# soasme/LTX-Video-GPUPoor

Measured on AMD Instinct MI355X. Metric: denoise-steps/sec + VAE-decode frames/sec, LTX-Video 768x512x97f at 1/8 GPU, higher is better.
Workload: dtype bf16

## Files before the change

### ltx-video-gpupoor_amd/ltxmi/attention.py

```python
from enum import Enum, auto
from typing import Optional

import torch
from torch import nn

from . import ff_mx8, lora, ops
from .attention_seam import pay_attention
from .derived import DerivedOwner, cache_key

BF16 = torch.bfloat16


FUSE_CROSS_ATTENTION_Q = True


class SkipLayerStrategy(Enum):
    AttentionSkip = auto()
    AttentionValues = auto()
    Residual = auto()
    TransformerBlock = auto()


def reshape_hidden_states(hidden_states, latent_frames):
    return hidden_states.reshape(hidden_states.shape[0], latent_frames, -1, hidden_states.shape[-1])


def restore_hidden_states_shape(hidden_states):
    return hidden_states.reshape(hidden_states.shape[0], -1, hidden_states.shape[-1])


class RMSNorm(nn.Module):

    def __init__(self, dim, eps: float, elementwise_affine: bool = True):
        super().__init__()
        self.eps = eps
        self.dim = dim
        if elementwise_affine:
            self.weight = nn.Parameter(torch.ones(dim))
        else:
            self.register_parameter("weight", None)


class _NoAffineLayerNorm(nn.Module):
    def __init__(self, dim, eps: float, elementwise_affine: bool = False):
        super().__init__()
        if elementwise_affine:
            raise NotImplementedError("ltxmi: standardisation norms with affine parameters are not on this path")
        self.eps = eps
        self.dim = dim


class GELUProj(nn.Module):

    def __init__(self, dim_in, dim_out, approximate="tanh", bias=True):
        super().__init__()
        self.proj = nn.Linear(dim_in, dim_out, bias=bias)
        self.approximate = approximate


class FeedForward(nn.Module):

    def __init__(self, dim, dim_out=None, mult=4, dropout=0.0, activation_fn="geglu", final_dropout=False,
                 inner_dim=None, bias=True):
        super().__init__()
        if activation_fn != "gelu-approximate":
            raise NotImplementedError(f"ltxmi: activation_fn '{activation_fn}' is not on this path "
# ... 126 lines not shown
                ops.rmsnorm_rope_(q2, attn.q_norm.weight, attn.q_norm.eps, cos, sin, period)
                ops.rmsnorm_rope_(k2, attn.k_norm.weight, attn.k_norm.eps, cos, sin, period)
            Lk = N
            q4 = qkv.view(B, N, 3, H, dh)[:, :, 0]
            k4 = qkv.view(B, N, 3, H, dh)[:, :, 1]
            v4 = qkv.view(B, N, 3, H, dh)[:, :, 2]
            v3 = qkv.view(B, N, 3 * D)[:, :, 2 * D:]
        else:
            Bk, Lk, _ = encoder_hidden_states.shape
            fuse_q = FUSE_CROSS_ATTENTION_Q and D % 64 == 0 and bool(ops.attention_fuses_qnorm(B, H, N, Lk, dh, attention_mask is not None))
            ss = torch.empty((B * N, D // 64), dtype=torch.float32, device=x2.device) if fuse_q else None
            q2 = ops.gemm(x2, attn.to_q.weight, attn.to_q.bias, rowsumsq=ss, rowsumsq_cols=D if fuse_q else 0,
                          **lora.pair(attn, "q", x2))
            ehs = encoder_hidden_states
            kv = None
            ready = attn.__dict__.get("_text_kv_ready")
            if ready is not None:
                full, full_key, kv_full, ready_epoch = ready
                row_bytes = full.stride(0) * full.element_size()
                off = ehs.data_ptr() - full.data_ptr()
                if (row_bytes > 0 and off >= 0 and off % row_bytes == 0 and ehs.shape[1:] == full.shape[1:]
                        and off // row_bytes + Bk <= full.shape[0] and ehs.dtype == full.dtype and ehs.is_contiguous()
                        and cache_key((full,)) == full_key and ready_epoch == lora.epoch(attn)):
                    r0 = off // row_bytes
                    kv = kv_full[r0 * Lk:(r0 + Bk) * Lk]
            if kv is None:
                def project():
                    e2 = ehs.reshape(Bk * Lk, -1)
                    kv = ops.gemm(e2, wkv, bkv, **lora.pair(attn, "kv", e2))
                    ops.rmsnorm_rope_(kv[:, :D], attn.k_norm.weight, attn.k_norm.eps)
                    return kv
                kv = attn.derived("text_kv", 4, True).get((ehs, wkv, attn.k_norm.weight), (lora.epoch(attn),), project,
                                                    enabled=ops.STEP_INVARIANT_CACHING)
            if fuse_q:
                q_fused = ((ops.rowsumsq_rstd(ss, D, attn.q_norm.eps), attn.q_norm.weight, attn.q_norm.eps), None)
            else:
                ops.rmsnorm_rope_(q2, attn.q_norm.weight, attn.q_norm.eps)
            q4 = q2.view(B, N, H, dh)
            k4 = kv.view(Bk, Lk, 2, H, dh)[:, :, 0]
            v4 = kv.view(Bk, Lk, 2, H, dh)[:, :, 1]
            v3 = kv.view(Bk, Lk, 2 * D)[:, :, D:]

        host_mask = _host_mask(skip_layer_mask) if skip_layer_mask is not None else None
        skip_attention = (host_mask is not None and skip_layer_strategy == SkipLayerStrategy.AttentionValues
                          and len(host_mask) == 1 and host_mask[0] == 0)
        if skip_attention:
            a3 = v3.contiguous()
        else:
            mask4 = None
            if attention_mask is not None:
                if attention_mask.dim() != 3 or attention_mask.shape[1] != 1:
                    raise NotImplementedError("ltxmi.AttnProcessor2_0: attention_mask must be a [B,1,Lk] bias")
                mask4 = attention_mask.reshape(B, 1, 1, Lk)
            a4 = self.attend([q4, k4, v4], is_cross, attention_mask=mask4, softmax_scale=attn.scale,
                             q_norm=q_fused[0] if q_fused else None, rope=q_fused[1] if q_fused else None)
            a3 = a4.view(B, N, D)
            if host_mask is not None and any(m != 1.0 for m in host_mask):
                m_dev = skip_layer_mask.reshape(B).to(torch.float32)
                if skip_layer_strategy == SkipLayerStrategy.AttentionValues:
                    ops.stg_blend_(a3, v3, m_dev)
                elif skip_layer_strategy == SkipLayerStrategy.AttentionSkip:
                    ops.stg_blend_(a3, hidden_states, m_dev)

        w_o, b_o = attn.to_out[0].weight, attn.to_out[0].bias
        if fused_residual is not None:
            residual, gate_table, gate_temb, rpg = fused_residual
            ops.gemm(a3.reshape(B * N, D), w_o, b_o, out=residual.reshape(B * N, -1),
                     epilogue=ops.EPI_GATE_RESIDUAL, residual=residual.reshape(B * N, -1),
                     gate_table=gate_table, gate_temb=gate_temb, rows_per_group=rpg,
                     **lora.pair(attn, "out", a3.reshape(B * N, D)))
            return residual
        out = ops.gemm(a3.reshape(B * N, D), w_o, b_o, **lora.pair(attn, "out", a3.reshape(B * N, D))).view(B, N, -1)
        if attn.residual_connection or attn.rescale_output_factor != 1.0:
            raise NotImplementedError("ltxmi.AttnProcessor2_0: residual_connection / rescale_output_factor")
        return out


class BasicTransformerBlock(nn.Module):

    def __init__(self, dim, num_attention_heads, attention_head_dim, dropout=0.0, cross_attention_dim=None,
                 activation_fn="geglu", num_embeds_ada_norm=None, attention_bias=False, only_cross_attention=False,
                 double_self_attention=False, upcast_attention=False, norm_elementwise_affine=True,
                 adaptive_norm="single_scale_shift", standardization_norm="layer_norm", norm_eps=1e-5,
                 qk_norm=None, final_dropout=False, attention_type="default", ff_inner_dim=None, ff_bias=True,
                 attention_out_bias=True, use_tpu_flash_attention=False, use_rope=False):
        super().__init__()
        if adaptive_norm != "single_scale_shift" or only_cross_attention or double_self_attention:
            raise NotImplementedError("ltxmi.BasicTransformerBlock: only the AdaLN-Zero "
                                      "(single_scale_shift) self+cross block is on this path")
        assert standardization_norm in ("layer_norm", "rms_norm")
        self.adaptive_norm = adaptive_norm
        self.norm_kind = ops.NORM_RMS if standardization_norm == "rms_norm" else ops.NORM_LAYER
        make_norm = RMSNorm if standardization_norm == "rms_norm" else _NoAffineLayerNorm
        if norm_elementwise_affine:
            raise NotImplementedError("ltxmi.BasicTransformerBlock: norm_elementwise_affine=True is not on this path")
        self.norm1 = make_norm(dim, eps=norm_eps, elementwise_affine=False)
        self.attn1 = Attention(query_dim=dim, heads=num_attention_heads, dim_head=attention_head_dim,
                               dropout=dropout, bias=attention_bias, cross_attention_dim=None,
                               out_bias=attention_out_bias, qk_norm=qk_norm, use_rope=use_rope)
        if cross_attention_dim is not None:
            self.attn2 = Attention(query_dim=dim, cross_attention_dim=cross_attention_dim,
                                   heads=num_attention_heads, dim_head=attention_head_dim, dropout=dropout,
                                   bias=attention_bias, out_bias=attention_out_bias, qk_norm=qk_norm,
                                   use_rope=use_rope)
        else:
            self.attn2 = None
        self.norm2 = make_norm(dim, norm_eps, False)
        self.ff = FeedForward(dim, dropout=dropout, activation_fn=activation_fn, final_dropout=final_dropout,
# ... 122 lines not shown
```

### ltx-video-gpupoor_amd/ltxmi/attention_seam.py

```python
import torch

from . import ops
from .derived import DerivedCache


def _key_bias_from_mask(attention_mask, B, Lk):
    m = attention_mask
    if m.dim() != 4 or m.shape[0] != B or m.shape[-1] != Lk:
        raise ValueError(f"pay_attention: attention_mask must be [B, 1|Lq, 1|H, Lk], got {tuple(m.shape)}")
    for d in (1, 2):
        if m.shape[d] != 1 and m.stride(d) != 0:
            raise NotImplementedError(
                "pay_attention: only key biases broadcast over queries and heads are supported "
                f"(mask dim {d} has size {m.shape[d]} with stride {m.stride(d)})")
    return _BIAS_CACHE.get((m,), (), lambda: m[:, 0, 0, :].to(torch.float32).contiguous())


_BIAS_CACHE = DerivedCache(4)


@torch.compiler.disable()
def pay_attention(qkv_list, dropout_p=0., softmax_scale=None, causal=False, window_size=(-1, -1),
                  deterministic=False, version=None, force_attention=None, attention_mask=None,
                  cross_attn=False, q_lens=None, k_lens=None, q_norm=None, rope=None):
    q, k, v = qkv_list
    qkv_list.clear()
    if (q_norm is not None or rope is not None) and (q_lens is not None or k_lens is not None):
        raise NotImplementedError("pay_attention: q_norm / rope on load with q_lens / k_lens")
    if causal or tuple(window_size) != (-1, -1) or dropout_p != 0.:
        raise NotImplementedError("pay_attention: causal / windowed / dropout attention is not on this path")
    if force_attention not in (None, "sdpa"):
        raise NotImplementedError(f"pay_attention: backend '{force_attention}' does not exist here (single HIP backend)")
    out_dtype = q.dtype
    if v.dtype != torch.bfloat16:
        raise TypeError(f"pay_attention: bf16 only on this path, got {v.dtype}")
    q = q.to(v.dtype)
    k = k.to(v.dtype)
    b, lq, lk = q.size(0), q.size(1), k.size(1)
    final_padding = 0

    if b > 1 and k_lens is not None:
        assert attention_mask is None and q_lens is None
        k_lens = [int(x) for x in k_lens]
        chunk_sizes, k_sizes = [], []
        cur, cnt = k_lens[0], 1
        for kl in k_lens[1:]:
            if kl == cur:
                cnt += 1
            else:
                chunk_sizes.append(cnt)
                k_sizes.append(cur)
                cur, cnt = kl, 1
        chunk_sizes.append(cnt)
        k_sizes.append(cur)
        if len(chunk_sizes) > 1 or k_lens[0] != k.shape[1]:
            outs = []
            for sq, sk, sv, sz in zip(torch.split(q, chunk_sizes), torch.split(k, chunk_sizes),
                                      torch.split(v, chunk_sizes), k_sizes):
                outs.append(pay_attention([sq, sk[:, :sz], sv[:, :sz]], softmax_scale=softmax_scale))
            return torch.cat(outs, dim=0)
    elif q_lens is not None or k_lens is not None:
        assert b == 1
        szq = int(q_lens[0]) if q_lens is not None else lq
        szk = int(k_lens[0]) if k_lens is not None else lk
        final_padding = lq - szq
        q, k, v = q[:, :szq], k[:, :szk], v[:, :szk]

    bias = None if attention_mask is None else _key_bias_from_mask(attention_mask, b, k.size(1))
    x = ops.attention(q, k, v, key_bias=bias, softmax_scale=softmax_scale, q_norm=q_norm, rope=rope)
    x = x.type(out_dtype)
    if final_padding > 0:
        x = torch.cat([x, torch.empty((x.shape[0], final_padding, *x.shape[-2:]), dtype=x.dtype, device=x.device)], 1)
    return x
```

### ltx-video-gpupoor_amd/ltxmi/ops.py

```python
import ctypes
import math

import torch

from . import _lib, _lib_mx, derived
from ._lib import lib, check

BF16 = torch.bfloat16


def _header(*names):
    return tuple(_lib.CONSTANTS["LTXMI_" + n] for n in names)


EPI_NONE, EPI_GELU_TANH, EPI_SILU, EPI_GATE_RESIDUAL = _header("EPI_NONE", "EPI_GELU_TANH", "EPI_SILU", "EPI_GATE_RESIDUAL")
NORM_RMS, NORM_LAYER = _header("NORM_RMS", "NORM_LAYER")


def _stream():
    return ctypes.c_void_p(torch.cuda.current_stream().cuda_stream)


_watch = None
_events = {}


def watch_launches(keys):
    global _watch
    _watch = set(keys) if keys else None
    _events.clear()


_redo_counter = None


def count_attention_redos(counter):
    global _redo_counter
    _redo_counter = counter


def launch_times_ms():
    return {k: [a.elapsed_time(b) for a, b in v] for k, v in _events.items()}


def _prof_begin(key, key2=None):
    if _watch is None:
        return None
    if key not in _watch:
        if key2 is None or key2 not in _watch:
            return None
        key = key2
    e0, e1 = torch.cuda.Event(enable_timing=True), torch.cuda.Event(enable_timing=True)
    e0.record()
    return key, e0, e1


def _prof_end(tok):
    if tok is not None:
# ... 134 lines not shown

def _norm_modulate(what, f32in, x, out, eps, kind, scale_table, scale_temb, shift_table, shift_temb, rows_per_group):
    if f32in:
        _chk_f32(x, what)
    _chk_bf16(None if f32in else x, out, scale_table, scale_temb, shift_table, shift_temb)
    x2, rows, ldx = _rows(x)
    o2, orows, ldy = _rows(out)
    D = x2.shape[1]
    if f32in and (orows != rows or o2.shape[1] != D):
        raise ValueError(f"ltxmi.{what}: out must have x's rows and channels")
    if scale_temb.stride(0) != shift_temb.stride(0):
        raise ValueError(f"ltxmi.{what}: scale/shift tables must share a row stride")
    entry = lib.ltxmi_norm_modulate_f32in_bf16 if f32in else lib.ltxmi_norm_modulate_bf16
    check(entry(_ptr(x2), ldx, _ptr(o2), ldy, rows, D, eps, kind, _ptr(scale_table), _ptr(scale_temb), _ptr(shift_table),
                _ptr(shift_temb), scale_temb.stride(0), rows_per_group, _stream()),
          "ltxmi_norm_modulate_f32in_bf16" if f32in else "ltxmi_norm_modulate_bf16")
    return out


def norm_modulate(x, out, eps, kind, scale_table, scale_temb, shift_table, shift_temb, rows_per_group):
    return _norm_modulate("norm_modulate", False, x, out, eps, kind, scale_table, scale_temb, shift_table, shift_temb,
                          rows_per_group)


def norm_modulate_f32in(x, out, eps, kind, scale_table, scale_temb, shift_table, shift_temb, rows_per_group):
    return _norm_modulate("norm_modulate_f32in", True, x, out, eps, kind, scale_table, scale_temb, shift_table, shift_temb,
                          rows_per_group)


def gate_residual_f32_(h, y, gate_table=None, gate_temb=None, rows_per_group=1, round_product=0, h_bf16=None):
    _chk_f32(h, "gate_residual_f32_")
    _chk_bf16(y, gate_table, gate_temb, h_bf16)
    h2, rows, ldh = _rows(h)
    y2, yrows, ldy = _rows(y)
    D = h2.shape[1]
    if yrows != rows or y2.shape[1] != D:
        raise ValueError("ltxmi.gate_residual_f32_: y must have h's rows and channels")
    if (gate_table is None) != (gate_temb is None):
        raise ValueError("ltxmi.gate_residual_f32_: gate_table and gate_temb go together")
    gate_ld = 0
    if gate_temb is not None:
        gate_ld = gate_temb.stride(0) if gate_temb.dim() == 2 else 0
    b2, ldb = None, 0
    if h_bf16 is not None:
        b2, brows, ldb = _rows(h_bf16)
        if brows != rows or b2.shape[1] != D:
            raise ValueError("ltxmi.gate_residual_f32_: h_bf16 must have h's rows and channels")
    check(lib.ltxmi_gate_residual_f32(_ptr(h2), ldh, _ptr(y2), ldy, rows, D, _ptr(gate_table), _ptr(gate_temb), gate_ld,
                                      rows_per_group, int(round_product), _ptr(b2), ldb, _stream()),
          "ltxmi_gate_residual_f32")
    return h


def rmsnorm_rope_(x, weight, eps, cos=None, sin=None, rope_period=0, rstd_of=None):
    _chk_bf16(x, weight, cos, sin)
    x2, rows, ldx = _rows(x)
    D = x2.shape[1]
    ld_tab = 0
    if cos is not None:
        if cos.dim() != 2 or cos.shape != sin.shape or cos.stride(0) != sin.stride(0):
            raise ValueError("ltxmi.rmsnorm_rope_: cos/sin must be matching 2-D tables")
        ld_tab = cos.stride(0)
        rope_period = rope_period or cos.shape[0]
    if rstd_of is not None:
        ss, norm_dim, norm_eps, out = rstd_of
        if ss.dtype != torch.float32 or out.dtype != torch.float32 or ss.dim() != 2 or ss.shape[0] != rows or \
                ss.stride(1) != 1 or out.shape != (rows,) or not out.is_contiguous():
            raise ValueError("ltxmi.rmsnorm_rope_: rstd_of needs fp32 sums [rows, blocks] and a contiguous fp32 out [rows]")
        check(lib.ltxmi_rmsnorm_rope_rstd_bf16(_ptr(x2), ldx, rows, D, _ptr(weight), eps, _ptr(cos), _ptr(sin), ld_tab,
                                               rope_period, _ptr(ss), ss.stride(0), ss.shape[1], norm_dim, norm_eps,
                                               _ptr(out), _stream()), "ltxmi_rmsnorm_rope_rstd_bf16")
        return x
    check(lib.ltxmi_rmsnorm_rope_bf16(_ptr(x2), ldx, rows, D, _ptr(weight), eps, _ptr(cos), _ptr(sin), ld_tab,
                                      rope_period, _stream()), "ltxmi_rmsnorm_rope_bf16")
    return x


def rowsumsq_rstd(ss, norm_dim, eps, out=None):
    if ss.dtype != torch.float32 or ss.dim() != 2 or ss.stride(1) != 1 or not ss.is_cuda:
        raise ValueError("ltxmi.rowsumsq_rstd: expected CUDA fp32 sums [rows, blocks]")
    rows = ss.shape[0]
    out = torch.empty((rows,), dtype=torch.float32, device=ss.device) if out is None else out
    check(lib.ltxmi_rowsumsq_rstd_f32(_ptr(ss), ss.stride(0), ss.shape[1], rows, norm_dim, eps, _ptr(out), _stream()),
          "ltxmi_rowsumsq_rstd_f32")
    return out


def attention_fuses_qnorm(B, H, Lq, Lk, dh, has_key_bias=False):
    return bool(lib.ltxmi_attention_fuses_qnorm(B, H, Lq, Lk, dh, int(has_key_bias)))


def attention_kernel_id(B, H, Lq, Lk, dh, has_key_bias=False, k_stride_l=None, v_stride_l=None):
    ks = 3 * H * dh if k_stride_l is None else k_stride_l
    vs = ks if v_stride_l is None else v_stride_l
    return int(lib.ltxmi_attention_kernel_id(B, H, Lq, Lk, dh, int(has_key_bias), ks, vs))


def _attn_shared(a, what, cuda_bias, dims, q, k, v, out, key_bias, softmax_scale):
    B, H, Lq, Lk, dh = dims
    a.q, a.q_stride_b, a.q_stride_l = q.data_ptr(), q.stride(0), q.stride(1)
    a.k, a.k_stride_b, a.k_stride_l = k.data_ptr(), k.stride(0), k.stride(1)
    a.v, a.v_stride_b, a.v_stride_l = v.data_ptr(), v.stride(0), v.stride(1)
    a.o, a.o_stride_b, a.o_stride_l = out.data_ptr(), out.stride(0), out.stride(1)
    if key_bias is not None:
        if key_bias.dtype != torch.float32 or key_bias.shape != (B, Lk) or key_bias.stride(1) != 1 \
                or (cuda_bias and not key_bias.is_cuda):
            raise ValueError(f"ltxmi.{what}: key_bias must be {'a CUDA ' if cuda_bias else ''}fp32 [B, Lk]")
        a.key_bias, a.bias_stride_b = key_bias.data_ptr(), key_bias.stride(0)
    a.B, a.H, a.Lq, a.Lk, a.head_dim = B, H, Lq, Lk, dh
    a.softmax_scale = softmax_scale


def _chk_attn_qkv(what, q, k, v, out):
    _chk_bf16(q, k, v, out)
    B, Lq, H, dh = q.shape
    for t in (q, k, v):
        if t.stride(3) != 1 or t.stride(2) != dh:
            raise ValueError(f"ltxmi.{what}: (heads, head_dim) must be contiguous")
    return B, H, Lq, k.shape[1], dh


# ... 7 lines not shown
    if out.dim() != 4 or out.stride(3) != 1 or out.stride(2) != dh:
        raise ValueError("ltxmi.attention: out must be 4-D with (heads, head_dim) contiguous")
    a = _lib.AttnArgs()
    if out_segments is not None:
        seg_len, seg_stride = out_segments
        if seg_len <= 0 or Lq % seg_len != 0 or tuple(out.shape) != (B, seg_len, H, dh):
            raise ValueError(f"ltxmi.attention: out_segments=({seg_len}, {seg_stride}) needs Lq={Lq} to be a multiple of the "
                             f"segment and out to be segment 0's [B, segment, H, dh] view, got {tuple(out.shape)}")
        a.o_segment_len, a.o_stride_segment = seg_len, seg_stride
    elif tuple(out.shape) != (B, Lq, H, dh):
        raise ValueError(f"ltxmi.attention: out must be [B, Lq, H, dh] = {(B, Lq, H, dh)}, got {tuple(out.shape)}")
    _attn_shared(a, "attention", False, dims, q, k, v, out, key_bias,
                 softmax_scale if softmax_scale is not None else 1.0 / math.sqrt(dh))
    if q_norm is not None:
        ss, w, eps = q_norm
        nb = H * dh // 64
        _chk_bf16(w)
        if ss.dim() == 1:
            if ss.dtype != torch.float32 or ss.shape != (B * Lq,) or ss.stride(0) != 1 or not ss.is_cuda:
                raise ValueError("ltxmi.attention: q_norm row factors must be a contiguous fp32 [B*Lq]")
            a.q_rstd, a.q_rstd_stride_b, a.q_rstd_stride_l = ss.data_ptr(), Lq, 1
        else:
            if ss.dtype != torch.float32 or ss.dim() != 2 or ss.shape != (B * Lq, nb) or ss.stride(1) != 1:
                raise ValueError("ltxmi.attention: q_norm row sums must be fp32 [B*Lq, H*dh/64]")
            a.q_rowsumsq, a.q_rowsumsq_stride_b, a.q_rowsumsq_stride_l = ss.data_ptr(), Lq * ss.stride(0), ss.stride(0)
            a.q_rowsumsq_blocks = nb
        a.q_norm_weight, a.q_norm_eps = w.data_ptr(), eps
        if rope is not None:
            cos, sin, period = rope
            _chk_bf16(cos, sin)
            if period not in (Lq, B * Lq) or cos.stride(0) != sin.stride(0) or cos.stride(1) != 1:
                raise ValueError("ltxmi.attention: rope tables must be [Lq or B*Lq, H*dh] with one row stride")
            a.rope_cos, a.rope_sin = cos.data_ptr(), sin.data_ptr()
            a.rope_stride_l = cos.stride(0)
            a.rope_stride_b = 0 if period == Lq else Lq * cos.stride(0)
    elif rope is not None:
        raise ValueError("ltxmi.attention: rope needs q_norm")
    if redo_counter is None:
        redo_counter = _redo_counter
    if redo_counter is not None:
        if redo_counter.dtype != torch.int32 or redo_counter.numel() != 1 or not redo_counter.is_cuda:
            raise ValueError("ltxmi.attention: redo_counter must be a CUDA int32 tensor of one element")
        a.redo_counter = redo_counter.data_ptr()
    a.force_exact = int(bool(force_exact))
    if return_lse or lse is not None:
        if lse is None:
            lse = torch.empty((B, H, Lq), dtype=torch.float32, device=q.device)
        _chk_lse(lse, B, H, Lq, "ltxmi.attention: lse")
        a.lse, a.lse_stride_b, a.lse_stride_h = lse.data_ptr(), lse.stride(0), lse.stride(1)
    tok = _prof_begin(("attention", B, H, Lq, Lk, dh))
    check(lib.ltxmi_attention_fwd_bf16(ctypes.byref(a), _stream()), "ltxmi_attention_fwd_bf16")
    _prof_end(tok)
    return (out, lse) if lse is not None else out


def _chk_lse(lse, B, H, Lq, what):
    if lse.dtype != torch.float32 or not lse.is_cuda or tuple(lse.shape) != (B, H, Lq) or lse.stride(2) != 1:
        raise ValueError(f"{what} must be a CUDA fp32 [B, H, Lq] = {(B, H, Lq)} tensor with contiguous tokens")


def attention_merge(outs, lses, out=None, return_lse=False, lse=None):
    n = len(outs)
    if n != len(lses) or not 2 <= n <= _lib.ATTN_MERGE_MAX:
        raise ValueError(f"ltxmi.attention_merge: {n} outputs / {len(lses)} lse tensors, need 2 .. {_lib.ATTN_MERGE_MAX} of each")
    _chk_bf16(*outs, out)
    B, Lq, H, dh = outs[0].shape
    if out is None:
        out = torch.empty((B, Lq, H, dh), dtype=BF16, device=outs[0].device)
    a = _lib.AttnMergeArgs()
    a.n = n
    for i, (o, l) in enumerate(zip(outs, lses)):
        if tuple(o.shape) != (B, Lq, H, dh) or o.stride(3) != 1 or o.stride(2) != dh:
            raise ValueError("ltxmi.attention_merge: partial outputs must be [B, Lq, H, dh] with (heads, head_dim) contiguous")
        _chk_lse(l, B, H, Lq, f"ltxmi.attention_merge: lses[{i}]")
        a.o_part[i], a.o_part_stride_b[i], a.o_part_stride_l[i] = o.data_ptr(), o.stride(0), o.stride(1)
        a.lse_part[i], a.lse_part_stride_b[i], a.lse_part_stride_h[i] = l.data_ptr(), l.stride(0), l.stride(1)
    if tuple(out.shape) != (B, Lq, H, dh) or out.stride(3) != 1 or out.stride(2) != dh:
        raise ValueError("ltxmi.attention_merge: out must be [B, Lq, H, dh] with (heads, head_dim) contiguous")
    a.o, a.o_stride_b, a.o_stride_l = out.data_ptr(), out.stride(0), out.stride(1)
    if return_lse or lse is not None:
        if lse is None:
            lse = torch.empty((B, H, Lq), dtype=torch.float32, device=out.device)
        _chk_lse(lse, B, H, Lq, "ltxmi.attention_merge: lse")
        a.lse, a.lse_stride_b, a.lse_stride_h = lse.data_ptr(), lse.stride(0), lse.stride(1)
    a.B, a.H, a.Lq, a.head_dim = B, H, Lq, dh
    check(lib.ltxmi_attention_merge_bf16(ctypes.byref(a), _stream()), "ltxmi_attention_merge_bf16")
    return (out, lse) if lse is not None else out


def qkv_norm_rope_pack(qkv, B, Nl, D, P, q_weight, k_weight, eps, cos=None, sin=None, rope_period=0, out=None):
    _chk_bf16(qkv, q_weight, k_weight, cos, sin, out)
    x2, rows, ld = _rows(qkv)
    if rows != B * Nl or x2.shape[1] != 3 * D:
        raise ValueError("ltxmi.qkv_norm_rope_pack: qkv must be [B*Nl, 3D]")
    if out is None:
        out = torch.empty((P, Nl, B, 3, D // P), dtype=BF16, device=qkv.device)
    if not out.is_contiguous() or out.numel() != rows * 3 * D:
        raise ValueError("ltxmi.qkv_norm_rope_pack: out must be a contiguous [P, Nl, B, 3, D/P] buffer")
    ld_tab = cos.stride(0) if cos is not None else 0
    check(lib.ltxmi_qkv_norm_rope_pack_bf16(_ptr(x2), ld, B, Nl, D, P, _ptr(q_weight), _ptr(k_weight), eps, _ptr(cos),
                                            _ptr(sin), ld_tab, rope_period, _ptr(out), _stream()),
          "ltxmi_qkv_norm_rope_pack_bf16")
    return out


def stg_blend_grouped_(a, v, m_f32):
# ... 560 lines not shown
```

Measured before the change: 16.50.

## Add cross-attention kernel that skips masked key tiles, plus shared-rope rmsnorm path

Adds a dedicated cross-attention kernel for head_dim 64 and short text keys. A small kernel counts, per batch, how many 64-key tiles hold unmasked keys, and that count is cached per bias tensor. The attention kernel loads only those tiles into shared memory and folds the q RMS-norm into its loads, so padded text tokens cost no matmul work. A separate RMSNorm+RoPE variant is also added that reuses rope tables when the row count is a multiple of the rope period. Both paths are new native kernels and bring risks: edge cases around the discard threshold, and a bias cache keyed on tensor identity.

```diff
diff --git a/include/ltxmi_dit.h b/include/ltxmi_dit.h
--- /dev/null
+++ b/include/ltxmi_dit.h
@@ -0,0 +1,41 @@
+#ifndef LTXMI_DIT_H
+#define LTXMI_DIT_H
+
+#include "ltxmi.h"
+
+#ifdef __cplusplus
+extern "C" {
+#endif
+
+#define LTXMI_DIT_VERSION "1"
+#define LTXMI_KEY_TILE 64
+#define LTXMI_KEY_DISCARD_AT -9000
+#define LTXMI_CROSS_TILES_MAX_KEYS 256
+
+int ltxmi_key_tile_count_f32(const float* key_bias, int64_t bias_stride_b, int32_t B, int32_t Lk, int32_t* key_tiles,
+                             void* stream);
+
+typedef struct ltxmi_cross_tiles_args {
+    const void* q; int64_t q_stride_b, q_stride_l;
+    const void* k; int64_t k_stride_b, k_stride_l;
+    const void* v; int64_t v_stride_b, v_stride_l;
+    void*       o; int64_t o_stride_b, o_stride_l;
+    const float* key_bias; int64_t bias_stride_b;
+    const int32_t* key_tiles;
+    const float* q_rstd; int64_t q_rstd_stride_b, q_rstd_stride_l;
+    const void* q_norm_weight;
+    int32_t B, H, Lq, Lk, head_dim;
+    float softmax_scale;
+} ltxmi_cross_tiles_args;
+
+int ltxmi_attention_cross_tiles_bf16(const ltxmi_cross_tiles_args* args, void* stream);
+
+int ltxmi_rmsnorm_rope_shared_bf16(void* x, int64_t ldx, int32_t B, int32_t N, int32_t D, const void* weight, float eps,
+                                   const void* cos_tab, const void* sin_tab, int64_t ld_tab, const float* rowsumsq,
+                                   int64_t rowsumsq_ld, int32_t rowsumsq_blocks, int32_t norm_dim, float norm_eps,
+                                   float* rstd_out, void* stream);
+
+#ifdef __cplusplus
+}
+#endif
+#endif
diff --git a/ltx-video-gpupoor_amd/csrc/attention_cross_tiles.hip b/ltx-video-gpupoor_amd/csrc/attention_cross_tiles.hip
--- /dev/null
+++ b/ltx-video-gpupoor_amd/csrc/attention_cross_tiles.hip
@@ -0,0 +1,318 @@
+#include "attention.h"
+#include "../../include/ltxmi_dit.h"
+
+namespace ltxmi {
+
+namespace cross_tiles {
+
+#ifndef LTXMI_XATTN_STAGGER
+#define LTXMI_XATTN_STAGGER 32
+#endif
+
+constexpr int DH = 64;
+constexpr int KV_TILE = LTXMI_KEY_TILE;
+constexpr int MAX_TILES = LTXMI_CROSS_TILES_MAX_KEYS / KV_TILE;
+constexpr int ROW_BYTES = DH * 2;
+constexpr int TILE_BYTES = KV_TILE * DH * 2;
+constexpr int K_OFF = 0, V_OFF = MAX_TILES * TILE_BYTES, BIAS_OFF = 2 * MAX_TILES * TILE_BYTES;
+constexpr int SCR_OFF = BIAS_OFF + MAX_TILES * KV_TILE * 16;
+constexpr int SCR_BYTES = 32 * 64;
+constexpr int QW_OFF = SCR_OFF + 4 * SCR_BYTES;
+constexpr int SMEM = QW_OFF + DH * 2;
+constexpr int ROWS_PER_IT = 128;
+constexpr float LOG2E = 1.4426950408889634f;
+
+__device__ __forceinline__ int k_swz(int row) { return (row >> 1) & 7; }
+
+template <int NT>
+__device__ __forceinline__ void attend(const AttnParams& p, char* smem, int b, int head, int row_begin, int row_end,
+                                       int stagger_from) {
+    const int tid = threadIdx.x;
+    const int lane = tid & 63;
+    const int wave = __builtin_amdgcn_readfirstlane(tid >> 6);
+    const int r = lane & 31, hh = lane >> 5;
+    const int n_it = (row_end - row_begin + ROWS_PER_IT - 1) / ROWS_PER_IT;
+
+    const uint16_t* qb = p.q + (int64_t)b * p.q_sb + head * DH;
+    const uint16_t* kb_ = p.k + (int64_t)b * p.k_sb + head * DH;
+    const uint16_t* vb = p.v + (int64_t)b * p.v_sb + head * DH;
+    uint16_t* ob = p.o + (int64_t)b * p.o_sb + head * DH;
+
+    {
+        u32x4 kreg[NT][2], vreg[NT][2];
+#pragma unroll
+        for (int t = 0; t < NT; ++t) {
+#pragma unroll
+            for (int i = 0; i < 2; ++i) {
+                const int c = tid + 256 * i;
+                int key = t * KV_TILE + (c >> 3);
+                key = key < p.Lk ? key : p.Lk - 1;
+                kreg[t][i] = *(const u32x4*)(kb_ + (int64_t)key * p.k_sl + (c & 7) * 8);
+                vreg[t][i] = *(const u32x4*)(vb + (int64_t)key * p.v_sl + (c & 7) * 8);
+            }
+        }
+        if (tid < NT * KV_TILE) {
+            float bv = ATTN_BIAS_FLOOR;
+            if (tid < p.Lk) bv = fmaxf(p.bias[(int64_t)b * p.bias_sb + tid] * (LOG2E / p.scale_log2e), ATTN_BIAS_FLOOR);
+            const __bf16 hi = (__bf16)bv;
+            const __bf16 lo = (__bf16)(bv - (float)hi);
+            u32x4 w = {0u, 0u, 0u, 0u};
+            w[0] = (uint32_t)__builtin_bit_cast(uint16_t, hi) | ((uint32_t)__builtin_bit_cast(uint16_t, lo) << 16);
+            *(u32x4*)(smem + BIAS_OFF + tid * 16) = w;
+        }
+#pragma unroll
+        for (int t = 0; t < NT; ++t) {
+#pragma unroll
+            for (int i = 0; i < 2; ++i) {
+                const int c = tid + 256 * i;
+                const int key = c >> 3, dc = c & 7;
+                *(u32x4*)(smem + K_OFF + t * TILE_BYTES + key * ROW_BYTES + ((dc ^ k_swz(key)) << 4)) = kreg[t][i];
+                *(u32x4*)(smem + V_OFF + t * TILE_BYTES + ((key >> 3) * 2 + (dc >> 2)) * 512 + (key & 7) * 64 + (dc & 3) * 16) = vreg[t][i];
+            }
+        }
+    }
+    if (tid < 8) *(u32x4*)(smem + QW_OFF + tid * 16) = *(const u32x4*)(p.q_w + head * DH + tid * 8);
+    __syncthreads();
+
+    const int k_rd0 = r * ROW_BYTES, k_rd1 = (32 + r) * ROW_BYTES;
+    const int k_sw0 = k_swz(r);
+    const int v_rd = attn_vt_offset(lane);
+    const bf16x8 ones = attn_ones_operand(lane);
+    const float c = p.scale_log2e;
+    char* scr = smem + SCR_OFF + wave * SCR_BYTES;
+
+    bf16x8 qraw[4], qf[4];
+    float q_rstd = 0.f;
+    auto load_q = [&](int it) {
+        const int row = row_begin + it * ROWS_PER_IT + wave * 32 + r;
+        const int q_ld = row < p.Lq ? row : p.Lq - 1;
+#pragma unroll
+        for (int s = 0; s < 4; ++s) qraw[s] = *(const bf16x8*)(qb + (int64_t)q_ld * p.q_sl + 16 * s + 8 * hh);
+        q_rstd = p.q_rstd[(int64_t)b * p.q_rstd_sb + (int64_t)q_ld * p.q_rstd_sl];
+    };
+    auto finish_q = [&]() {
+#pragma unroll
+        for (int s = 0; s < 4; ++s) {
+            const bf16x8 wv = *(const bf16x8*)(smem + QW_OFF + (16 * s + 8 * hh) * 2);
+#pragma unroll
+            for (int e = 0; e < 8; ++e) qf[s][e] = (__bf16)((float)qraw[s][e] * q_rstd * (float)wv[e]);
+        }
+    };
+    load_q(0);
+    finish_q();
+    if (n_it > 1) load_q(1);
+    if (blockIdx.x >= (unsigned)stagger_from) __builtin_amdgcn_s_sleep(LTXMI_XATTN_STAGGER);
+
+    for (int it = 0; it < n_it; ++it) {
+        const int q0 = row_begin + it * ROWS_PER_IT + wave * 32;
+
+        constexpr int NG = 2 * NT;
+        f32x16 sT[NG];
+        bf16x8 kfr[5];
+        bf16x8 qaug;
+        {
+            uint32_t w0 = hh == 0 ? 0x3f803f80u : 0u, w1 = 0u;
+            asm volatile("" : "+v"(w0), "+v"(w1));
+            const u32x4 w = {w0, w1, w1, w1};
+            qaug = __builtin_bit_cast(bf16x8, w);
+        }
+        auto read_k1 = [&](int g, int j) {
+            if (j == 0) {
+                kfr[0] = *(const bf16x8*)(smem + BIAS_OFF + (32 * g + r) * 16);
+            } else {
+                const char* ks = smem + K_OFF + (g >> 1) * TILE_BYTES + ((g & 1) ? k_rd1 : k_rd0);
+                kfr[j] = *(const bf16x8*)(ks + (((2 * (j - 1) + hh) ^ k_sw0) << 4));
+            }
+        };
+        auto max3 = [](float a, float b2, float c3) { return fmaxf(fmaxf(a, b2), c3); };
+        float mt = -INFINITY;
+        auto group_max = [&](int g) {
+            const f32x16& x = sT[g];
+            const float a = max3(x[0], x[1], x[2]), b2 = max3(x[3], x[4], x[5]), c2 = max3(x[6], x[7], x[8]);
+            const float d2 = max3(x[9], x[10], x[11]), e2 = max3(x[12], x[13], x[14]);
+            mt = max3(max3(a, b2, c2), max3(d2, e2, x[15]), mt);
+            asm volatile("" : "+v"(mt));
+        };
+#pragma unroll
+        for (int j = 0; j < 5; ++j) read_k1(0, j);
+#pragma unroll
+        for (int g = 0; g < NG; ++g) {
+#pragma unroll
+            for (int j = 0; j < 5; ++j) {
+                if (j == 0) {
+                    const f32x16 z16 = {0.f, 0.f, 0.f, 0.f, 0.f, 0.f, 0.f, 0.f, 0.f, 0.f, 0.f, 0.f, 0.f, 0.f, 0.f, 0.f};
+                    sT[g] = __builtin_amdgcn_mfma_f32_32x32x16_bf16(kfr[0], qaug, z16, 0, 0, 0);
+                } else {
+                    sT[g] = __builtin_amdgcn_mfma_f32_32x32x16_bf16(kfr[j], qf[j - 1], sT[g], 0, 0, 0);
+                }
+                if (g + 1 < NG) read_k1(g + 1, j);
+                __builtin_amdgcn_sched_barrier(0);
+            }
+            if (g >= 1) group_max(g - 1);
+        }
+        if (it + 1 < n_it) finish_q();
+        if (it + 2 < n_it) load_q(it + 2);
+        group_max(NG - 1);
+        mt = attn_lane_half_max(mt);
+        const float nmc = -mt * c;
+
+        f32x16 oT[2];
+        f32x4 lT;
+        const f32x16 z16 = {0.f, 0.f, 0.f, 0.f, 0.f, 0.f, 0.f, 0.f, 0.f, 0.f, 0.f, 0.f, 0.f, 0.f, 0.f, 0.f};
+        const f32x4 z4 = {0.f, 0.f, 0.f, 0.f};
+        auto read_v = [&](int t, int sp, bf16x8 (&dst)[2]) {
+            const char* vs = smem + V_OFF + t * TILE_BYTES + v_rd;
+#pragma unroll
+            for (int d = 0; d < 2; ++d)
+                dst[d] = attn_vt_fragment<DH>(vs + (2 * sp * 2 + d) * 512);
+        };
+        auto make_p = [&](int t, int sp2, bf16x8& dst) {
+            const f32x16& x = sT[2 * t + (sp2 >> 1)];
+            const f32x2 c2v = {c, c}, m2v = {nmc, nmc};
+#pragma unroll
+            for (int e = 0; e < 8; e += 2) {
+                const f32x2 y = f32x2{x[8 * (sp2 & 1) + e], x[8 * (sp2 & 1) + e + 1]} * c2v + m2v;
+                dst[e] = (__bf16)fast_exp2(y[0]);
+                dst[e + 1] = (__bf16)fast_exp2(y[1]);
+            }
+            asm volatile("" : "+v"(dst));
+        };
+        bf16x8 pfr[2][4], vfr[2][2];
+#pragma unroll
+        for (int sp = 0; sp < 4; ++sp) make_p(0, sp, pfr[0][sp]);
+        read_v(0, 0, vfr[0]);
+#pragma unroll
+        for (int t = 0; t < NT; ++t) {
+#pragma unroll
+            for (int sp = 0; sp < 4; ++sp) {
+                const int st = 4 * t + sp;
+                if (st + 1 < 4 * NT) read_v((st + 1) >> 2, (st + 1) & 3, vfr[(st + 1) & 1]);
+                const bf16x8& pf = pfr[t & 1][sp];
+                lT = __builtin_amdgcn_mfma_f32_16x16x32_bf16(ones, pf, st == 0 ? z4 : lT, 0, 0, 0);
+                oT[0] = __builtin_amdgcn_mfma_f32_32x32x16_bf16(vfr[st & 1][0], pf, st == 0 ? z16 : oT[0], 0, 0, 0);
+                oT[1] = __builtin_amdgcn_mfma_f32_32x32x16_bf16(vfr[st & 1][1], pf, st == 0 ? z16 : oT[1], 0, 0, 0);
+                if (t + 1 < NT) make_p(t + 1, sp, pfr[(t + 1) & 1][sp]);
+                __builtin_amdgcn_sched_barrier(0);
+            }
+        }
+
+        const float l0 = __shfl(lT[0], r & 15, 64), l1v = __shfl(lT[1], r & 15, 64);
+        const float lrow = (r & 16) ? l1v : l0;
+        const float inv = 1.0f / lrow;
+#pragma unroll
+        for (int d = 0; d < 2; ++d) {
+#pragma unroll
+            for (int g = 0; g < 4; ++g) {
+                u32x2 w;
+                w[0] = pack_bf16(oT[d][4 * g + 0] * inv, oT[d][4 * g + 1] * inv);
+                w[1] = pack_bf16(oT[d][4 * g + 2] * inv, oT[d][4 * g + 3] * inv);
+                *(u32x2*)(scr + r * 64 + ((g ^ (r & 3)) << 4) + hh * 8) = w;
+            }
+#pragma unroll
+            for (int t2 = 0; t2 < 2; ++t2) {
+                const int row = t2 * 16 + (lane >> 2), chunk = lane & 3;
+                const u32x4 w = *(const u32x4*)(scr + row * 64 + ((chunk ^ (row & 3)) << 4));
+                if (q0 + row < row_end) *(u32x4*)(ob + (int64_t)(q0 + row) * p.o_sl + 32 * d + chunk * 8) = w;
+            }
+        }
+    }
+}
+
+__global__ __launch_bounds__(256, 2) void attn_cross_tiles_kernel(AttnParams p, const int* __restrict__ key_tiles, int groups,
+                                                                  int rows_per_group, int stagger_from) {
+    extern __shared__ __attribute__((aligned(16))) char smem[];
+    const int work = xcd_work_id();
+    const int bh = work / groups, grp = work % groups;
+    const int b = bh / p.H, head = bh % p.H;
+    const int row_begin = grp * rows_per_group;
+    const int row_end = min(p.Lq, row_begin + rows_per_group);
+    if (row_begin >= row_end) return;
+    const int full = (p.Lk + KV_TILE - 1) / KV_TILE;
+    const int nt = min(max(__builtin_amdgcn_readfirstlane(key_tiles[b]), 1), full);
+    switch (nt) {
+        case 1: attend<1>(p, smem, b, head, row_begin, row_end, stagger_from); break;
+        case 2: attend<2>(p, smem, b, head, row_begin, row_end, stagger_from); break;
+        case 3: attend<3>(p, smem, b, head, row_begin, row_end, stagger_from); break;
+        default: attend<4>(p, smem, b, head, row_begin, row_end, stagger_from); break;
+    }
+}
+
+__global__ __launch_bounds__(64) void key_tile_count_kernel(const float* __restrict__ bias, int64_t bias_sb, int Lk,
+                                                            int* __restrict__ key_tiles) {
+    const int b = blockIdx.x, lane = threadIdx.x;
+    int last = -1;
+    for (int j = lane; j < Lk; j += 64) {
+        const uint32_t bits = __float_as_uint(bias[(int64_t)b * bias_sb + j]);
+        const bool nan = (bits & 0x7fffffffu) > 0x7f800000u;
+        if (nan || __uint_as_float(bits) > (float)LTXMI_KEY_DISCARD_AT) last = j;
+    }
+#pragma unroll
+    for (int o = 32; o > 0; o >>= 1) last = max(last, __shfl_xor(last, o, 64));
+    if (lane == 0) key_tiles[b] = last >= 0 ? last / KV_TILE + 1 : (Lk + KV_TILE - 1) / KV_TILE;
+}
+
+}
+
+}
+
+using namespace ltxmi;
+
+extern "C" int ltxmi_key_tile_count_f32(const float* key_bias, int64_t bias_stride_b, int32_t B, int32_t Lk, int32_t* key_tiles,
+                                        void* stream) {
+    LTXMI_REQUIRE(key_bias && key_tiles, LTXMI_ERR_INVALID_ARG, "ltxmi_key_tile_count_f32: NULL argument");
+    LTXMI_REQUIRE(B > 0 && Lk > 0, LTXMI_ERR_INVALID_ARG, "ltxmi_key_tile_count_f32: non-positive size B=%d Lk=%d", B, Lk);
+    LTXMI_REQUIRE(B == 1 || bias_stride_b >= Lk, LTXMI_ERR_INVALID_ARG,
+                  "ltxmi_key_tile_count_f32: bias_stride_b=%lld is shorter than a row of Lk=%d", (long long)bias_stride_b, Lk);
+    LTXMI_REQUIRE(((((uintptr_t)key_bias) | ((uintptr_t)key_tiles)) & 3) == 0, LTXMI_ERR_INVALID_ARG,
+                  "ltxmi_key_tile_count_f32: key_bias and key_tiles must be 4-byte aligned");
+    hipLaunchKernelGGL(cross_tiles::key_tile_count_kernel, dim3((unsigned)B), dim3(64), 0, (hipStream_t)stream, key_bias,
+                       bias_stride_b, Lk, key_tiles);
+    return check_launch("ltxmi_key_tile_count_f32");
+}
+
+extern "C" int ltxmi_attention_cross_tiles_bf16(const ltxmi_cross_tiles_args* a, void* stream) {
+    const char* what = "ltxmi_attention_cross_tiles_bf16";
+    LTXMI_REQUIRE(a && a->q && a->k && a->v && a->o && a->key_bias && a->key_tiles && a->q_rstd && a->q_norm_weight,
+                  LTXMI_ERR_INVALID_ARG, "%s: NULL argument", what);
+    LTXMI_REQUIRE(a->B > 0 && a->H > 0 && a->Lq > 0 && a->Lk > 0, LTXMI_ERR_INVALID_ARG,
+                  "%s: non-positive shape B=%d H=%d Lq=%d Lk=%d", what, a->B, a->H, a->Lq, a->Lk);
+    LTXMI_REQUIRE(((((uintptr_t)a->key_bias) | ((uintptr_t)a->key_tiles) | ((uintptr_t)a->q_rstd)) & 3) == 0 &&
+                      (((uintptr_t)a->q_norm_weight) & 15) == 0,
+                  LTXMI_ERR_INVALID_ARG, "%s: key_bias, key_tiles, q_rstd must be 4-byte and q_norm_weight 16-byte aligned", what);
+    LTXMI_REQUIRE(a->head_dim == cross_tiles::DH, LTXMI_ERR_UNSUPPORTED, "%s: head_dim %d is not 64", what, a->head_dim);
+    LTXMI_REQUIRE(a->Lk <= LTXMI_CROSS_TILES_MAX_KEYS, LTXMI_ERR_UNSUPPORTED, "%s: Lk=%d is more than %d keys", what, a->Lk,
+                  LTXMI_CROSS_TILES_MAX_KEYS);
+    const int64_t strides[] = {a->q_stride_b, a->q_stride_l, a->k_stride_b, a->k_stride_l,
+                               a->v_stride_b, a->v_stride_l, a->o_stride_b, a->o_stride_l};
+    for (int64_t s : strides) LTXMI_REQUIRE(s % 8 == 0, LTXMI_ERR_UNSUPPORTED, "%s: strides must be multiples of 8 elements", what);
+    LTXMI_REQUIRE((((uintptr_t)a->q | (uintptr_t)a->k | (uintptr_t)a->v | (uintptr_t)a->o) & 15) == 0, LTXMI_ERR_UNSUPPORTED,
+                  "%s: q/k/v/o must be 16-byte aligned", what);
+    LTXMI_REQUIRE((int64_t)a->B * a->H * ((a->Lq + cross_tiles::ROWS_PER_IT - 1) / cross_tiles::ROWS_PER_IT) < (1ll << 31),
+                  LTXMI_ERR_UNSUPPORTED, "%s: grid too large", what);
+    AttnParams p = {};
+    p.q = (const uint16_t*)a->q; p.q_sb = a->q_stride_b; p.q_sl = a->q_stride_l;
+    p.k = (const uint16_t*)a->k; p.k_sb = a->k_stride_b; p.k_sl = a->k_stride_l;
+    p.v = (const uint16_t*)a->v; p.v_sb = a->v_stride_b; p.v_sl = a->v_stride_l;
+    p.o = (uint16_t*)a->o; p.o_sb = a->o_stride_b; p.o_sl = a->o_stride_l;
+    p.bias = a->key_bias; p.bias_sb = a->bias_stride_b;
+    p.B = a->B; p.H = a->H; p.Lq = a->Lq; p.Lk = a->Lk;
+    p.scale_log2e = a->softmax_scale * 1.4426950408889634f;
+    p.q_rstd = a->q_rstd; p.q_rstd_sb = a->q_rstd_stride_b; p.q_rstd_sl = a->q_rstd_stride_l;
+    p.q_w = (const uint16_t*)a->q_norm_weight;
+
+    const int n_cu = device_cu_count(what);
+    if (n_cu <= 0) return LTXMI_ERR_LAUNCH;
+    const int slots = 2 * n_cu, bh = p.B * p.H;
+    int groups = slots / bh;
+    if (groups < 1) groups = 1;
+    const int max_groups = (p.Lq + 2 * cross_tiles::ROWS_PER_IT - 1) / (2 * cross_tiles::ROWS_PER_IT);
+    if (groups > max_groups) groups = max_groups;
+    int rows = (p.Lq + groups - 1) / groups;
+    rows = (rows + cross_tiles::ROWS_PER_IT - 1) / cross_tiles::ROWS_PER_IT * cross_tiles::ROWS_PER_IT;
+    groups = (p.Lq + rows - 1) / rows;
+    static unsigned long long lds_done = 0;
+    if (const int rc = reserve_lds((const void*)cross_tiles::attn_cross_tiles_kernel, cross_tiles::SMEM, &lds_done, what)) return rc;
+    hipLaunchKernelGGL(cross_tiles::attn_cross_tiles_kernel, dim3((unsigned)((int64_t)bh * groups)), dim3(256), cross_tiles::SMEM,
+                       (hipStream_t)stream, p, (const int*)a->key_tiles, groups, rows, n_cu);
+    return check_launch(what);
+}
diff --git a/ltx-video-gpupoor_amd/csrc/rmsnorm_rope_shared.hip b/ltx-video-gpupoor_amd/csrc/rmsnorm_rope_shared.hip
--- /dev/null
+++ b/ltx-video-gpupoor_amd/csrc/rmsnorm_rope_shared.hip
@@ -0,0 +1,89 @@
+#include "rows.h"
+#include "../../include/ltxmi_dit.h"
+
+namespace ltxmi {
+
+template <int NCH>
+__global__ __launch_bounds__(256) void rmsnorm_rope_shared_kernel(uint16_t* __restrict__ x, int64_t ldx, int B, int N, int D,
+                                                                  const uint16_t* __restrict__ w, float eps,
+                                                                  const uint16_t* __restrict__ cs,
+                                                                  const uint16_t* __restrict__ sn, int64_t ld_tab,
+                                                                  const float* __restrict__ side_ss, int64_t side_ld, int side_n,
+                                                                  float side_inv_d, float side_eps,
+                                                                  float* __restrict__ side_rstd) {
+    const int lane = threadIdx.x & 63;
+    const int g = __builtin_amdgcn_readfirstlane(blockIdx.x * ROWS_PER_WG + (threadIdx.x >> 6));
+    const int n = g / B;
+    if (n >= N) return;
+    const int row = (g - n * B) * N + n;
+    if (side_ss) {
+        float t = 0.f;
+        for (int j = lane; j < side_n; j += 64) t += side_ss[(int64_t)row * side_ld + j];
+        t = wave_sum(t);
+        if (lane == 0) side_rstd[row] = rsqrtf(t * side_inv_d + side_eps);
+    }
+    const int nchunk = D >> 3;
+    uint16_t* xr = x + (int64_t)row * ldx;
+    Chunk c[NCH];
+    float s2 = 0.f;
+    LTXMI_FOR_ROW_CHUNKS(NCH, lane, nchunk, j, ch) {
+        c[j] = load_bf16x8(xr + ch * 8);
+#pragma unroll
+        for (int e = 0; e < 8; ++e) s2 += c[j].v[e] * c[j].v[e];
+    }
+    s2 = wave_sum(s2);
+    const float rstd = rsqrtf(s2 / D + eps);
+    const int64_t trow = cs ? (int64_t)n * ld_tab : 0;
+    LTXMI_FOR_ROW_CHUNKS(NCH, lane, nchunk, j, ch) {
+        const Chunk wt = load_bf16x8(w + ch * 8);
+        Chunk o;
+#pragma unroll
+        for (int e = 0; e < 8; ++e) o.v[e] = c[j].v[e] * rstd * wt.v[e];
+        if (cs) {
+            const Chunk co = load_bf16x8(cs + trow + ch * 8), si = load_bf16x8(sn + trow + ch * 8);
+            Chunk r2;
+#pragma unroll
+            for (int e = 0; e < 8; e += 2) {
+                r2.v[e] = o.v[e] * co.v[e] - o.v[e + 1] * si.v[e];
+                r2.v[e + 1] = o.v[e + 1] * co.v[e + 1] + o.v[e] * si.v[e + 1];
+            }
+            o = r2;
+        }
+        store_bf16x8(xr + ch * 8, o);
+    }
+}
+
+}
+
+using namespace ltxmi;
+
+extern "C" int ltxmi_rmsnorm_rope_shared_bf16(void* x, int64_t ldx, int32_t B, int32_t N, int32_t D, const void* weight, float eps,
+                                              const void* cos_tab, const void* sin_tab, int64_t ld_tab, const float* rowsumsq,
+                                              int64_t rowsumsq_ld, int32_t rowsumsq_blocks, int32_t norm_dim, float norm_eps,
+                                              float* rstd_out, void* stream) {
+    const char* what = "ltxmi_rmsnorm_rope_shared_bf16";
+    LTXMI_REQUIRE(x && weight && cos_tab && sin_tab, LTXMI_ERR_INVALID_ARG, "%s: NULL argument", what);
+    LTXMI_REQUIRE(B > 0 && N > 0 && D > 0, LTXMI_ERR_INVALID_ARG, "%s: non-positive size B=%d N=%d D=%d", what, B, N, D);
+    if (rowsumsq || rstd_out)
+        LTXMI_REQUIRE(rowsumsq && rstd_out && rowsumsq_blocks > 0 && norm_dim > 0 && rowsumsq_ld >= rowsumsq_blocks &&
+                          ((((uintptr_t)rowsumsq) | ((uintptr_t)rstd_out)) & 3) == 0,
+                      LTXMI_ERR_INVALID_ARG, "%s: bad rowsumsq geometry (blocks %d, ld %lld, dim %d)", what, rowsumsq_blocks,
+                      (long long)rowsumsq_ld, norm_dim);
+    LTXMI_REQUIRE(D % 8 == 0 && D <= 2048, LTXMI_ERR_UNSUPPORTED, "%s: D=%d must be a multiple of 8 and <= 2048", what, D);
+    LTXMI_REQUIRE(row_stride_ok(ldx, D) && row_stride_ok(ld_tab, D), LTXMI_ERR_UNSUPPORTED,
+                  "%s: ldx=%lld and ld_tab=%lld must be multiples of 8 and cover D=%d", what, (long long)ldx, (long long)ld_tab, D);
+    LTXMI_REQUIRE(aligned16((const char*)x, (const char*)weight, (const char*)cos_tab, (const char*)sin_tab), LTXMI_ERR_UNSUPPORTED,
+                  "%s: x, weight, cos_tab and sin_tab must be 16-byte aligned", what);
+    LTXMI_REQUIRE((int64_t)B * N < (1ll << 31) - ROWS_PER_WG, LTXMI_ERR_UNSUPPORTED, "%s: B * N = %lld rows: the wave index reaches 2^31", what,
+                  (long long)B * N);
+    const int grid = (int)(((int64_t)B * N + ROWS_PER_WG - 1) / ROWS_PER_WG);
+    auto go = [&](auto nch) {
+        hipLaunchKernelGGL((rmsnorm_rope_shared_kernel<decltype(nch)::value>), dim3(grid), dim3(256), 0, (hipStream_t)stream,
+                           (uint16_t*)x, ldx, B, N, D, (const uint16_t*)weight, eps, (const uint16_t*)cos_tab,
+                           (const uint16_t*)sin_tab, ld_tab, rowsumsq, rowsumsq_ld, rowsumsq_blocks,
+                           1.0f / (float)(rowsumsq ? norm_dim : 1), norm_eps, rstd_out);
+    };
+    if (D <= 512) go(std::integral_constant<int, 1>{});
+    else go(std::integral_constant<int, 4>{});
+    return check_launch(what);
+}
diff --git a/ltx-video-gpupoor_amd/ltxmi/_lib_dit.py b/ltx-video-gpupoor_amd/ltxmi/_lib_dit.py
--- /dev/null
+++ b/ltx-video-gpupoor_amd/ltxmi/_lib_dit.py
@@ -0,0 +1,23 @@
+import os
+
+from . import _abi, _lib
+
+HEADER_PATH = os.path.join(os.path.dirname(_lib.HEADER_PATH), "ltxmi_dit.h")
+STRUCT_NAMES = {"ltxmi_cross_tiles_args": "CrossTilesArgs"}
+
+if not os.path.exists(HEADER_PATH):
+    raise ImportError(f"ltxmi: {HEADER_PATH} is missing -- the DiT-step binding is read from it. There is no fallback path.")
+with open(HEADER_PATH) as _f:
+    ABI = _abi.parse(_f.read(), STRUCT_NAMES)
+lib = _lib.lib
+for _name, (_res, _args) in ABI.signatures.items():
+    _fn = getattr(lib, _name)
+    _fn.restype = _res
+    _fn.argtypes = _args
+globals().update(ABI.structs)
+SIGNATURES = ABI.signatures
+CONSTANTS = ABI.constants
+DIT_VERSION = ABI.strings["LTXMI_DIT_VERSION"]
+KEY_TILE = CONSTANTS["LTXMI_KEY_TILE"]
+CROSS_TILES_MAX_KEYS = CONSTANTS["LTXMI_CROSS_TILES_MAX_KEYS"]
+check = _lib.check
diff --git a/ltx-video-gpupoor_amd/ltxmi/attention.py b/ltx-video-gpupoor_amd/ltxmi/attention.py
--- a/ltx-video-gpupoor_amd/ltxmi/attention.py
+++ b/ltx-video-gpupoor_amd/ltxmi/attention.py
@@ -12,6 +12,7 @@
 
 
 FUSE_CROSS_ATTENTION_Q = True
+CROSS_KEY_TILES = True
 
 
 class SkipLayerStrategy(Enum):
@@ -244,8 +245,13 @@
                 if attention_mask.dim() != 3 or attention_mask.shape[1] != 1:
                     raise NotImplementedError("ltxmi.AttnProcessor2_0: attention_mask must be a [B,1,Lk] bias")
                 mask4 = attention_mask.reshape(B, 1, 1, Lk)
+            extra = {}
+            if (is_cross and CROSS_KEY_TILES and mask4 is not None and q_fused is not None and q_fused[1] is None
+                    and q_fused[0][0].dim() == 1 and k4.shape[0] == B
+                    and ops.cross_tiles_applies(B, H, N, Lk, dh, k4.stride(1), v4.stride(1))):
+                extra["key_tiles"] = True
             a4 = self.attend([q4, k4, v4], is_cross, attention_mask=mask4, softmax_scale=attn.scale,
-                             q_norm=q_fused[0] if q_fused else None, rope=q_fused[1] if q_fused else None)
+                             q_norm=q_fused[0] if q_fused else None, rope=q_fused[1] if q_fused else None, **extra)
             a3 = a4.view(B, N, D)
             if host_mask is not None and any(m != 1.0 for m in host_mask):
                 m_dev = skip_layer_mask.reshape(B).to(torch.float32)
diff --git a/ltx-video-gpupoor_amd/ltxmi/attention_seam.py b/ltx-video-gpupoor_amd/ltxmi/attention_seam.py
--- a/ltx-video-gpupoor_amd/ltxmi/attention_seam.py
+++ b/ltx-video-gpupoor_amd/ltxmi/attention_seam.py
@@ -17,12 +17,17 @@
 
 
 _BIAS_CACHE = DerivedCache(4)
+_TILES_CACHE = DerivedCache(4)
+
+
+def _key_tiles_of(bias):
+    return _TILES_CACHE.get((bias,), (), lambda: ops.key_tile_count(bias))
 
 
 @torch.compiler.disable()
 def pay_attention(qkv_list, dropout_p=0., softmax_scale=None, causal=False, window_size=(-1, -1),
                   deterministic=False, version=None, force_attention=None, attention_mask=None,
-                  cross_attn=False, q_lens=None, k_lens=None, q_norm=None, rope=None):
+                  cross_attn=False, q_lens=None, k_lens=None, q_norm=None, rope=None, key_tiles=False):
     q, k, v = qkv_list
     qkv_list.clear()
     if (q_norm is not None or rope is not None) and (q_lens is not None or k_lens is not None):
@@ -67,7 +72,12 @@
         q, k, v = q[:, :szq], k[:, :szk], v[:, :szk]
 
     bias = None if attention_mask is None else _key_bias_from_mask(attention_mask, b, k.size(1))
-    x = ops.attention(q, k, v, key_bias=bias, softmax_scale=softmax_scale, q_norm=q_norm, rope=rope)
+    if key_tiles:
+        if bias is None or q_norm is None or rope is not None or q_lens is not None or k_lens is not None:
+            raise ValueError("pay_attention: key_tiles needs attention_mask and q_norm, without rope / q_lens / k_lens")
+        x = ops.attention_cross_tiles(q, k, v, bias, _key_tiles_of(bias), q_norm, softmax_scale=softmax_scale)
+    else:
+        x = ops.attention(q, k, v, key_bias=bias, softmax_scale=softmax_scale, q_norm=q_norm, rope=rope)
     x = x.type(out_dtype)
     if final_padding > 0:
         x = torch.cat([x, torch.empty((x.shape[0], final_padding, *x.shape[-2:]), dtype=x.dtype, device=x.device)], 1)
diff --git a/ltx-video-gpupoor_amd/ltxmi/ops.py b/ltx-video-gpupoor_amd/ltxmi/ops.py
--- a/ltx-video-gpupoor_amd/ltxmi/ops.py
+++ b/ltx-video-gpupoor_amd/ltxmi/ops.py
@@ -3,7 +3,7 @@
 
 import torch
 
-from . import _lib, _lib_mx, derived
+from . import _lib, _lib_dit, _lib_mx, derived
 from ._lib import lib, check
 
 BF16 = torch.bfloat16
@@ -244,6 +244,16 @@
     return h
 
 
+SHARED_ROPE_ROWS = True
+
+
+def rmsnorm_rope_route(rows, D, ldx, has_rope, ld_tab, rope_period):
+    if (SHARED_ROPE_ROWS and has_rope and 0 < rope_period < rows and rows % rope_period == 0 and D % 8 == 0 and D <= 2048
+            and ldx >= D and ld_tab >= D):
+        return "shared"
+    return "rows"
+
+
 def rmsnorm_rope_(x, weight, eps, cos=None, sin=None, rope_period=0, rstd_of=None):
     _chk_bf16(x, weight, cos, sin)
     x2, rows, ldx = _rows(x)
@@ -259,6 +269,14 @@
         if ss.dtype != torch.float32 or out.dtype != torch.float32 or ss.dim() != 2 or ss.shape[0] != rows or \
                 ss.stride(1) != 1 or out.shape != (rows,) or not out.is_contiguous():
             raise ValueError("ltxmi.rmsnorm_rope_: rstd_of needs fp32 sums [rows, blocks] and a contiguous fp32 out [rows]")
+    if rmsnorm_rope_route(rows, D, ldx, cos is not None, ld_tab, rope_period) == "shared":
+        ss, norm_dim, norm_eps, out = rstd_of if rstd_of is not None else (None, 0, 0.0, None)
+        _lib_dit.check(_lib_dit.lib.ltxmi_rmsnorm_rope_shared_bf16(
+            _ptr(x2), ldx, rows // rope_period, rope_period, D, _ptr(weight), eps, _ptr(cos), _ptr(sin), ld_tab, _ptr(ss),
+            0 if ss is None else ss.stride(0), 0 if ss is None else ss.shape[1], norm_dim, norm_eps, _ptr(out), _stream()),
+            "ltxmi_rmsnorm_rope_shared_bf16")
+        return x
+    if rstd_of is not None:
         check(lib.ltxmi_rmsnorm_rope_rstd_bf16(_ptr(x2), ldx, rows, D, _ptr(weight), eps, _ptr(cos), _ptr(sin), ld_tab,
                                                rope_period, _ptr(ss), ss.stride(0), ss.shape[1], norm_dim, norm_eps,
                                                _ptr(out), _stream()), "ltxmi_rmsnorm_rope_rstd_bf16")
@@ -372,6 +390,57 @@
     check(lib.ltxmi_attention_fwd_bf16(ctypes.byref(a), _stream()), "ltxmi_attention_fwd_bf16")
     _prof_end(tok)
     return (out, lse) if lse is not None else out
+
+
+def key_tile_count(key_bias, out=None):
+    if key_bias.dtype != torch.float32 or key_bias.dim() != 2 or key_bias.stride(1) != 1 or not key_bias.is_cuda:
+        raise ValueError("ltxmi.key_tile_count: key_bias must be a CUDA fp32 [B, Lk] tensor with contiguous keys")
+    B, Lk = key_bias.shape
+    if out is None:
+        out = torch.empty((B,), dtype=torch.int32, device=key_bias.device)
+    elif out.dtype != torch.int32 or tuple(out.shape) != (B,) or not out.is_contiguous() or not out.is_cuda:
+        raise ValueError("ltxmi.key_tile_count: out must be a contiguous CUDA int32 [B]")
+    _lib_dit.check(_lib_dit.lib.ltxmi_key_tile_count_f32(_ptr(key_bias), key_bias.stride(0), B, Lk, _ptr(out), _stream()),
+                   "ltxmi_key_tile_count_f32")
+    return out
+
+
+ATTN_KERNEL_CROSS = 7
+
+
+def cross_tiles_applies(B, H, Lq, Lk, dh, k_stride_l=None, v_stride_l=None):
+    return dh == 64 and Lk <= _lib_dit.CROSS_TILES_MAX_KEYS and \
+        attention_kernel_id(B, H, Lq, Lk, dh, True, k_stride_l, v_stride_l) == ATTN_KERNEL_CROSS
+
+
+def attention_cross_tiles(q, k, v, key_bias, key_tiles, q_norm, softmax_scale=None, out=None):
+    B, H, Lq, Lk, dh = dims = _chk_attn_qkv("attention_cross_tiles", q, k, v, out)
+    if dh != 64:
+        raise ValueError(f"ltxmi.attention_cross_tiles: head_dim {dh} is not 64")
+    if out is None:
+        out = torch.empty((B, Lq, H, dh), dtype=BF16, device=q.device)
+    if tuple(out.shape) != (B, Lq, H, dh) or out.stride(3) != 1 or out.stride(2) != dh:
+        raise ValueError(f"ltxmi.attention_cross_tiles: out must be [B, Lq, H, dh] = {(B, Lq, H, dh)} with (heads, head_dim) contiguous")
+    if key_bias is None or not key_bias.is_cuda:
+        raise ValueError("ltxmi.attention_cross_tiles: key_bias must be a CUDA fp32 [B, Lk]")
+    if key_tiles.dtype != torch.int32 or tuple(key_tiles.shape) != (B,) or not key_tiles.is_contiguous() or not key_tiles.is_cuda:
+        raise ValueError("ltxmi.attention_cross_tiles: key_tiles must be a contiguous CUDA int32 [B]")
+    rstd, w, _eps = q_norm
+    _chk_bf16(w)
+    if rstd.dtype != torch.float32 or rstd.shape != (B * Lq,) or rstd.stride(0) != 1 or not rstd.is_cuda:
+        raise ValueError("ltxmi.attention_cross_tiles: q_norm row factors must be a contiguous CUDA fp32 [B*Lq]")
+    if w.shape != (H * dh,) or not w.is_contiguous():
+        raise ValueError("ltxmi.attention_cross_tiles: q_norm weight must be a contiguous [H*dh]")
+    a = _lib_dit.CrossTilesArgs()
+    _attn_shared(a, "attention_cross_tiles", True, dims, q, k, v, out, key_bias,
+                 softmax_scale if softmax_scale is not None else 1.0 / math.sqrt(dh))
+    a.key_tiles = key_tiles.data_ptr()
+    a.q_rstd, a.q_rstd_stride_b, a.q_rstd_stride_l = rstd.data_ptr(), Lq, 1
+    a.q_norm_weight = w.data_ptr()
+    tok = _prof_begin(("attention", B, H, Lq, Lk, dh))
+    _lib_dit.check(_lib_dit.lib.ltxmi_attention_cross_tiles_bf16(ctypes.byref(a), _stream()), "ltxmi_attention_cross_tiles_bf16")
+    _prof_end(tok)
+    return out
 
 
 def _chk_lse(lse, B, H, Lq, what):
```

Measured after the change: 16.61 (median of 6 runs). No clear change (+0.7%).
